# chalharu/rust-compression

Hardware: AMD Instinct MI355X
Metric: BZip2 level-9 encode MB/s (input bytes, HBM-resident in and out: the kernels' rate; value_end_to_end is host buffer to host buffer at the C ABI) (higher is better)
Workload: dtype u8/u32

## Files before the change

rust-compression_amd/csrc/bzgpu.h:

```cpp
#pragma once
#include <hip/hip_runtime.h>
#include <stdint.h>
#include <stddef.h>

namespace bzgpu {

typedef uint8_t u8;
typedef uint16_t u16;
typedef uint32_t u32;
typedef uint64_t u64;
typedef int64_t i64;

constexpr u32 kWave = 64;
constexpr u32 kMaxBlockLen = 900000;
constexpr u32 kSortTile = 8192;
constexpr u32 kSortThreads = 512;
constexpr u32 kTilesPerBlock = 110;
constexpr u32 kSlot = kTilesPerBlock * kSortTile;
constexpr u32 kPtSlot = kSlot / 8u * 10u;
constexpr u32 kPairWords = 65536u / 32u;
constexpr u32 kMaxBins = 2048;
constexpr u32 kPerK = 8;
constexpr u32 kGSize = 50;
constexpr u32 kMaxSelectors = 18002;
// ... 427 lines not shown
constexpr u32 kDecEntrySkip = 0xFFFFFFFFu;
struct DecEntry {
    u64 off, len;
    u32 first_cand, ncand;
};
enum : u32 { kChainOk = 0, kChainData = 1, kChainMagicFirst = 2, kChainMagic = 3 };
struct DecChainEntry {
    u32 verdict;
    u32 streams;
    u32 irregular;
    u32 ntrue;
};
struct DecChainCand {
    u32 is_true, max_len;
    u32 stored_crc, nsym;
};
void launch_dec_scan_batch(hipStream_t st, const u8 *in, u64 span0, u64 span_end, const DecEntry *ents, u32 nent,
                           DecCand *cands, u32 cap, u32 *count);
void launch_dec_blocks_batch(hipStream_t st, const u8 *in, const DecEntry *ents, const DecCand *cands, u32 ncand,
                             DecBlockInfo *info, u16 *sym, u8 *sel_scratch);
void launch_dec_chain_batch(hipStream_t st, const u8 *in, const DecEntry *ents, u32 e0, u32 ne, const DecCand *cands,
                            u32 cand0, const DecBlockInfo *info, DecChainEntry *out_ent, DecChainCand *out_cand);
void launch_dec_mtf(hipStream_t st, const DecArgs &a, KernelProf *prof, int *rec);
void launch_dec_gather_windows(hipStream_t st, const u8 *in, u64 nbytes, const u64 *bases, u32 nw, u8 *out);
void launch_dec_walks(hipStream_t st, const DecArgs &a, u32 walk_wgs, hipStream_t st2, hipEvent_t ev_a, hipEvent_t ev_b,
                      KernelProf *prof, int rec[4]);
void launch_dec_expand(hipStream_t st, const DecArgs &a, const u64 *out_base, u8 *out);
void launch_dec_crc(hipStream_t st, const DecArgs &a, const u64 *out_base, const u8 *out, u32 max_out_len,
                    const u32 *crc_tab, const u32 *xp2, const u32 *xp16);

enum KernelId {
    KID_RADIX_HIST = 0,
    KID_RADIX_SCAN,
    KID_RADIX_SCATTER,
    KID_GROUP_FLAGS,
    KID_GROUP_APPLY,
    KID_LAST_COLUMN,
    KID_RADIX_SCATTER_LB,
    KID_GHIST_TEXT,
    KID_GHIST_SCAN,
    KID_RANK_PLACE,
    KID_PHASE_B_LOCAL,
    KID_GROUP_REFINE,
    KID_DEC_BLOCK,
    KID_DEC_MTF,
    KID_DEC_TSORT,
    KID_DEC_WALK,
    KID_DEC_PLACE,
    KID_DEC_RLE,
    KID_DEC_CRC,
    KID_RLE_ONEPASS,
    KID_RLE_SCATTER,
    KID_MTF_HEADS,
    KID_COUNT
};
struct KernelProf {
    bool on = false;
    struct Rec {
        int id;
        u64 bytes;
        hipEvent_t a, b;
    };
    Rec *recs = nullptr;
    u32 nrecs = 0, cap = 0;
    u64 launches[KID_COUNT] = {};
    u64 bytes[KID_COUNT] = {};
    double seconds[KID_COUNT] = {};
    int begin(hipStream_t st, int id, u64 nbytes);
    void end(hipStream_t st, int idx);
    void set_bytes(int idx, u64 nbytes) { if (idx >= 0) recs[idx].bytes = nbytes; }
    void collect();
    void reset();
};

void launch_slab_last(hipStream_t st, const RleBuffers &rb, u64 t0, u64 t1, i64 *d_out);
void launch_rle_scan(hipStream_t st, const u8 *d_in, u64 n, u64 t0, u64 t1, u64 in_begin, const u32 *crc_tab,
                     const u32 *xp16, const RleBuffers &rb);
void launch_rle_count(hipStream_t st, const u8 *d_in, u64 n, u64 t0, u64 t1, u64 in_begin, i64 init_carry,
                      const RleBuffers &rb, i64 *d_out_last);
void launch_rle_prefix(hipStream_t st, u64 tb, u64 t1, const RleBuffers &rb, bool write_end = true);
void launch_rle_cuts(hipStream_t st, const u8 *d_in, u64 n, u64 tb, u64 t1, u64 in_begin, const RleBuffers &rb,
                     u32 block_max_len, int emit_tail, BlockDesc *d_blocks, u32 max_blocks);
void launch_rle_image(hipStream_t st, const u8 *d_in, u64 n, u64 tb, u64 t1, u64 in_begin, const RleBuffers &rb, u8 *d_rle);
u64 rle_onepass_spans(u64 ntiles);
u32 rle_onepass_epochs();
void launch_rle_onepass(hipStream_t st, const u8 *d_in, u64 n, u64 ntiles, u32 epoch, const u32 *crc_tab, const u32 *xp16,
                        const RleBuffers &rb, u8 *d_rle, i64 *d_out_last);
u64 cut_table_entries(const CutPlan &pl);
void cut_groups(const CutPlan &pl, u64 *g_lo, u64 *g_hi, u64 *entries);
u32 cut_seg_cap();
void launch_cut_steps(hipStream_t st, const CutPlan &pl, const RleBuffers &rb, const CutBuffers &cb);
void launch_cut_tables(hipStream_t st, const CutPlan &pl, const u8 *d_in, u64 n_lim, const RleBuffers &rb, const CutBuffers &cb,
                       u64 work_total);
void launch_cut_select(hipStream_t st, const CutPlan &pl, u64 j0, u64 s0, u64 start_in, u64 n, long long rle_bias, int emit_tail,
                       const RleBuffers &rb, const CutBuffers &cb, BlockDesc *d_blocks, u32 max_blocks);
void launch_block_crc(hipStream_t st, const u8 *d_in, const BlockDesc *d_blocks, u32 nblocks,
                      const u32 *crc_tab, const u32 *xp2, const u32 *tile_crc, u32 *d_crc);
void launch_rle_batch(hipStream_t st, const u8 *d_in, const RleBatchItem *d_items, u32 count, const u32 *crc_tab,
                      const u32 *xp2, u8 *d_rle, BlockDesc *d_blocks, u32 *d_crc);
void launch_block_symbols(hipStream_t st, const BwtArgs &a, u32 *inuse_bits, u8 *sym_code, u8 *keyinfo);
int run_bwt(hipStream_t st, const BwtArgs &a, u32 max_n, u64 total_n, unsigned long long *h_active,
            u64 *sorted_elems, KernelProf *prof, u64 *round_active , bool wide_keys,
            u32 min_chars);
void launch_mtf(hipStream_t st, const MtfArgs &a, KernelProf *prof = nullptr, u64 total_n = 0);
inline bool env_verify() { return getenv("BZ_VERIFY") && atoi(getenv("BZ_VERIFY")) != 0; }
struct MailSeg {
// ... 19 lines not shown
```

rust-compression_amd/csrc/engine.hip:

```cpp
#include "engine_state.h"

#include <algorithm>
#include <chrono>
#include <cstdio>
#include <cstdlib>
#include <cstring>
#include <vector>

#define MAILCHK(st, ...)                                                             \
    do {                                                                             \
        const MailSeg mail_segs_[] = {__VA_ARGS__};                                  \
        if (mail_fetch((st), mail_segs_, (int)(sizeof(mail_segs_) / sizeof(mail_segs_[0]))) != 0) return BZ_E_UNEXPECTED; \
    } while (0)

static int span_begin(bz_gpu_engine *g, int stage, hipStream_t st = nullptr)
{
    bz_gpu_engine::Span s;
    s.stage = stage;
    s.st = st ? st : g->st;
    if (hipEventCreate(&s.a) != hipSuccess || hipEventCreate(&s.b) != hipSuccess) return -1;
    (void)hipEventRecord(s.a, s.st);
    g->spans.push_back(s);
    return (int)g->spans.size() - 1;
}
// ... 1781 lines not shown
        if (bad) {
            fprintf(stderr, "bz2_mi355x: the one-launch ZLE stage misbehaved (tile tickets / look-back); stage redone with three kernels\n");
            g->zle_fused_broken = true;
            ma.fused_zle = 0;
            launch_mtf(g->st, ma, nullptr, total_n);
        }
    }
    std::vector<BlockOut> outs(nb);
    HIPCHK(hipMemcpyAsync(outs.data(), g->bout.p, nb * sizeof(BlockOut), hipMemcpyDeviceToHost, g->st));
    HIPCHK(hipMemcpyAsync(h_freq, g->mtf_freq.p, nb * kMaxAlpha * 4, hipMemcpyDeviceToHost, g->st));
    HIPCHK(hipStreamSynchronize(g->st));
    for (size_t i = 0; i < nb; ++i) {
        if (outs[i].mtf_count == 0 || outs[i].mtf_count > h_len[i] + 1u) return BZ_E_UNEXPECTED;
        h_mtf_count[i] = outs[i].mtf_count;
        h_in_use[i] = outs[i].in_use_count;
        HIPCHK(hipMemcpyAsync(h_sym + i * sym_stride, g->mtf.as<u16>() + i * kMtfStride, (size_t)outs[i].mtf_count * 2,
                              hipMemcpyDeviceToHost, g->st));
    }
    HIPCHK(hipStreamSynchronize(g->st));
    HIPCHK(hipGetLastError());
    return BZ_OK;
}

extern "C" int bz_gpu_debug_code_lengths(bz_gpu_engine *g, const uint32_t *h_freq, size_t alpha, uint8_t *h_len,
                                         int *took_length_limited_path)
{
    if (!g || alpha == 0 || alpha > kMaxAlpha) return BZ_E_PARAM;
    {
        uint64_t total = 0;
        for (size_t i = 0; i < alpha; ++i) total += h_freq[i] ? h_freq[i] : 1u;
        if (total >= (1u << 20)) return BZ_E_PARAM;
    }
    HIPCHK(hipSetDevice(g->device));
    DevBuf f, o, s, fl;
    int rc;
    if ((rc = f.ensure(alpha * 4)) || (rc = o.ensure(alpha + 8)) || (rc = s.ensure((size_t)kLmWords * 4)) ||
        (rc = fl.ensure(4)))
        return rc;
    HIPCHK(hipMemcpyAsync(f.p, h_freq, alpha * 4, hipMemcpyHostToDevice, g->st));
    launch_probe_code_lengths(g->st, f.as<u32>(), (u32)alpha, o.as<u8>(), s.as<u32>(), fl.as<int>());
    int flag = 0;
    HIPCHK(hipMemcpyAsync(h_len, o.p, alpha, hipMemcpyDeviceToHost, g->st));
    HIPCHK(hipMemcpyAsync(&flag, fl.p, 4, hipMemcpyDeviceToHost, g->st));
    HIPCHK(hipStreamSynchronize(g->st));
    HIPCHK(hipGetLastError());
    if (took_length_limited_path) *took_length_limited_path = flag;
    return BZ_OK;
}

static const char *kKernelNames[KID_COUNT] = {"k_radix_hist", "k_radix_scan", "k_radix_scatter",
                                              "k_group_flags", "k_group_apply", "k_last_column",
                                              "k_radix_scatter_lb", "k_ghist_text", "k_ghist_scan", "k_rank_place", "k_phase_b_local", "k_group_refine",
                                              "k_dec_block", "k_dec_mtf", "k_dec_tsort", "k_dec_walk_lengths",
                                              "k_dec_place", "k_dec_rle", "k_dec_crc", "k_rle_onepass", "k_rle_scatter", "k_mtf_heads"};

extern "C" int bz_gpu_profile_enable(bz_gpu_engine *g, int on)
{
    if (!g) return BZ_E_PARAM;
    g->prof.reset();
    g->prof.on = (on & 1) != 0;
    g->debug_figures = (on & 2) != 0;
    return BZ_OK;
}

extern "C" int bz_gpu_profile_kernels(bz_gpu_engine *g)
{
    (void)g;
    return KID_COUNT;
}

extern "C" int bz_gpu_profile_get(bz_gpu_engine *g, int idx, const char **name, uint64_t *launches,
                                  double *seconds, uint64_t *algorithmic_bytes)
{
    if (!g || idx < 0 || idx >= KID_COUNT) return BZ_E_PARAM;
    if (name) *name = kKernelNames[idx];
    if (launches) *launches = g->prof.launches[idx];
    if (seconds) *seconds = g->prof.seconds[idx];
    if (algorithmic_bytes) *algorithmic_bytes = g->prof.bytes[idx];
    return BZ_OK;
}
```

rust-compression_amd/csrc/k_bwt.hip:

```cpp
#include "bzgpu.h"
#include <algorithm>
#include <atomic>
#include <cstdio>
#include <cstdlib>
#include <vector>

namespace bzgpu {
constexpr u32 kGhSpan = 8;
constexpr u32 kSymSpan = 8;

enum { SRC_TEXT = 0, SRC_PAIRS = 1, SRC_MM = 2, SRC_WALK = 3, SRC_SURV = 4, SRC_LISTG = 5,
       SRC_TEXTK = 6, SRC_WALKK = 7, SRC_MMK = 8,
       SRC_MMC = 9,
       SRC_PERJ = 10,
       SRC_PACKED = 11,
       SRC_PERJK = 12,
       SRC_WALKA = 13 };
template <int SRC> struct src_is_list {
    static constexpr bool value = (SRC == SRC_PAIRS || SRC == SRC_SURV || SRC == SRC_LISTG || SRC == SRC_PERJ || SRC == SRC_PERJK || SRC == SRC_PACKED);
};

struct KeyInfo {
    u8 bits;
    u8 chars;
// ... 972 lines not shown
}

__device__ __forceinline__ void loc_fill(u64 (&e)[16], const u64 *s_e, u32 pos0, u32 len, u32 l, u64 le_mask, u32 gshift,
                                         u32 &gcarry)
{
#pragma unroll
    for (u32 r = 0; r < 16; ++r) {
        const u32 i = pos0 + r * 64u + l;
        const u64 x = s_e[i < len ? i : len - 1u];
        const u64 m = __ballot(i < len && (x >> 63) != 0);
        const u32 gi = gcarry + (u32)__popcll(m & le_mask) - 1u;
        e[r] = (x & ~(1ull << 63)) | ((u64)gi << gshift);
        gcarry += (u32)__popcll(m);
    }
}
__device__ __forceinline__ void loc_rank(const u64 (&e)[16], u32 (&rnk)[16], u32 *cnt, u32 pos0, u32 len, u32 l, u32 shift)
{
#pragma unroll
    for (u32 q = 0; q < kLocBins / 2 / 64; ++q) cnt[q * 64u + l] = 0;
#pragma unroll
    for (u32 r = 0; r < 16; ++r) {
        const u32 i = pos0 + r * 64u + l;
        const u32 dg = (u32)(e[r] >> shift) & (kLocBins - 1u);
        const u32 sh = (dg & 1u) * 16u;
        u32 old = 0;
        if (i < len)
            old = __hip_atomic_fetch_add(cnt + (dg >> 1), 1u << sh, __ATOMIC_RELAXED, __HIP_MEMORY_SCOPE_WORKGROUP);
        rnk[r] = (old >> sh) & 0xFFFFu;
    }
}
__device__ __forceinline__ void loc_move(const u64 (&e)[16], const u32 (&rnk)[16], const u32 *cnt, const u16 *s_tpre,
                                         u64 *s_e, u32 pos0, u32 len, u32 l, u32 shift)
{
    const u16 *c16 = reinterpret_cast<const u16 *>(cnt);
#pragma unroll
    for (u32 r = 0; r < 16; ++r) {
        const u32 i = pos0 + r * 64u + l;
        const u32 dg = (u32)(e[r] >> shift) & (kLocBins - 1u);
        const u32 to = (u32)s_tpre[dg] + (u32)c16[dg] + rnk[r];
        if (i < len) s_e[to] = e[r];
    }
}
__device__ __forceinline__ void loc_reload(u64 (&e)[16], const u64 *s_e, u32 pos0, u32 len, u32 l)
{
#pragma unroll
    for (u32 r = 0; r < 16; ++r) {
        const u32 i = pos0 + r * 64u + l;
        e[r] = s_e[i < len ? i : len - 1u];
    }
}

#define LOC_T(k) do { } while (0)
constexpr u32 LOC_STAT_SURV_FAIL = 80;
__device__ __forceinline__ u32 first_group_start_list(const u32 *__restrict__ R, const u32 *__restrict__ Vb, u32 p0, u32 cnt, u32 limit)
{
    if (p0 == 0) return 0;
    if (p0 >= cnt) return cnt;
    const u32 l = threadIdx.x & 63u;
    for (u32 q0 = p0; q0 < p0 + limit; q0 += 64u) {
        if (q0 >= cnt) return cnt;
        const u32 q = q0 + l;
        bool b = false;
        if (q < cnt) b = (R[Vb[q] & 0xFFFFFu] & ~kFinalBit) != (R[Vb[q - 1] & 0xFFFFFu] & ~kFinalBit);
        const u64 m = __ballot(b);
        if (m) return q0 + (u32)__ffsll((long long)m) - 1u;
    }
    return 0xFFFFFFFFu;
}
__global__ __launch_bounds__(kLocThreads) void k_surv_local(BwtArgs a, u32 step, const u32 *__restrict__ V, u32 *__restrict__ Kout,
                                                             u32 *__restrict__ Vout)
{
    __shared__ u64 s_e[kLocCap];
    __shared__ u32 s_cnt[kLocSets][kLocBins / 2];
    __shared__ u16 s_tpre[kLocBins];
    __shared__ u32 s_wsum[kLocSets];
    __shared__ u32 s_seg[2];
    __shared__ u32 s_bad;
    u32 tile, lb;
    xcd_remap(gridDim.x, a.nb, tile, lb);
    if (lb == 0xFFFFFFFFu) return;
    const u32 n = a.blocks[lb].n;
    const u32 cnt = a.count[lb];
    const u32 start = tile * kSortTile;
    if (start >= cnt) return;
    const KeyInfo ki = reinterpret_cast<const KeyInfo *>(a.keyinfo)[lb];
    const u32 hm = (((u32)ki.chars * 2u) << step) % n;
    const size_t base = (size_t)lb * kSlot;
    const u32 *Rb = a.R + base, *Vl = V + base;
    const u32 w = threadIdx.x >> 6, l = threadIdx.x & 63u;
    if (w == 0) {
        const u32 s = first_group_start_list(Rb, Vl, start, cnt, kLocCap + 64u);
        if (l == 0) s_seg[0] = s;
    } else if (w == 1) {
        const u32 s = first_group_start_list(Rb, Vl, start + kSortTile, cnt, kLocCap + 64u);
        if (l == 0) s_seg[1] = s;
    }
    if (threadIdx.x == 0) s_bad = 0;
    __syncthreads();
    const u32 s0 = (u32)__builtin_amdgcn_readfirstlane((int)s_seg[0]), s1 = (u32)__builtin_amdgcn_readfirstlane((int)s_seg[1]);
    if (s0 == 0xFFFFFFFFu || s1 == 0xFFFFFFFFu || (s1 > s0 && s1 - s0 > kLocCap)) {
        if (threadIdx.x == 0) atomicAdd(&a.loc_stats[LOC_STAT_SURV_FAIL], 1u);
        return;
    }
    if (s1 <= s0) return;
    const u32 len = s1 - s0;
    const u32 *Vb = Vl + s0;
    const u32 wu = (u32)__builtin_amdgcn_readfirstlane((int)w);
    const u32 posA = wu * 1024u, posB = kSortTile + wu * 1024u;
    u32 gcount[2] = {0, 0};
#pragma unroll 1
    for (u32 half = 0; half < 2; ++half) {
        const u32 pos0 = half ? posB : posA;
        if (pos0 >= len) break;
        u32 prev_last = 0;
        if (l == 0 && pos0 > 0) prev_last = Rb[Vb[pos0 - 1u] & 0xFFFFFu] & ~kFinalBit;
        const u32 rows = (len - pos0 + 63u) / 64u < 16u ? (len - pos0 + 63u) / 64u : 16u;
        u32 tot = 0;
#pragma unroll 4
        for (u32 r = 0; r < rows; ++r) {
            const u32 i = pos0 + r * 64u + l;
            const u32 c = i < len ? i : len - 1u;
            const u32 v = ld_stream(Vb + c) & 0xFFFFFu;
// ... 23 lines not shown
        groups += c;
    }
    const u64 le_mask = (l == 63) ? ~0ull : ((2ull << l) - 1ull);
    constexpr u32 kbits = 20u;
    const u32 gshift = 20u + kbits;
    const bool haveB = posB < len;
    u64 eA[16], eB[16];
    loc_fill(eA, s_e, posA, len, l, le_mask, gshift, gcarryA);
    if (haveB) loc_fill(eB, s_e, posB, len, l, le_mask, gshift, gcarryB);
    const u32 gbits = groups > 1u ? 32u - (u32)__builtin_clz(groups - 1u) : 0u;
    const u32 npass = (kbits + gbits + kLocBits - 1u) / kLocBits;
    u32 *cntA = s_cnt[w], *cntB = s_cnt[kLocWaves + w];
    u16 *cnt16 = reinterpret_cast<u16 *>(&s_cnt[0][0]);
#pragma unroll 1
    for (u32 p = 0; p < npass; ++p) {
        const u32 shift = 20u + p * kLocBits;
        u32 rnkA[16], rnkB[16];
        loc_rank(eA, rnkA, cntA, posA, len, l, shift);
        if (haveB) loc_rank(eB, rnkB, cntB, posB, len, l, shift);
        else {
#pragma unroll
            for (u32 q = 0; q < kLocBins / 2 / 64; ++q) cntB[q * 64u + l] = 0;
        }
        __syncthreads();
        u32 tot;
        {
            const u32 dg = threadIdx.x;
            u32 run = 0;
#pragma unroll
            for (u32 k = 0; k < kLocSets; ++k) {
                const u32 c = cnt16[k * kLocBins + dg];
                cnt16[k * kLocBins + dg] = (u16)run;
                run += c;
            }
            tot = run;
        }
        const u32 inc = wave_incl_sum(tot);
        if (l == 63) s_wsum[w] = inc;
        __syncthreads();
        {
            u32 carry = 0;
            for (u32 k = 0; k < w; ++k) carry += s_wsum[k];
            s_tpre[threadIdx.x] = (u16)(carry + inc - tot);
        }
        __syncthreads();
        loc_move(eA, rnkA, cntA, s_tpre, s_e, posA, len, l, shift);
        if (haveB) loc_move(eB, rnkB, cntB, s_tpre, s_e, posB, len, l, shift);
        __syncthreads();
        if (p + 1 < npass) {
            loc_reload(eA, s_e, posA, len, l);
            if (haveB) loc_reload(eB, s_e, posB, len, l);
        }
    }
    {
        bool bad = false;
        for (u32 i = threadIdx.x; i < len; i += kLocThreads) {
            const u64 x = s_e[i];
            if (i && (s_e[i - 1] >> 20) > (x >> 20)) bad = true;
            const u32 v = (u32)x & 0xFFFFFu;
            Vout[base + s0 + i] = v;
            Kout[base + s0 + i] = Rb[v] & ~kFinalBit;
        }
        if (__ballot(bad) && l == 0) s_bad = 1u;
    }
    __syncthreads();
    if (threadIdx.x == 0 && s_bad) atomicAdd(&a.loc_stats[LOC_STAT_SURV_FAIL], 1u);
}

template <bool INIT>
__global__ __launch_bounds__(kSortThreads) void k_group_flags(BwtArgs a, u32 step, const u32 *__restrict__ K,
                                                               const u32 *__restrict__ V,
                                                               const u8 *__restrict__ impure = nullptr)
{
    __shared__ int s_old, s_new;
    u32 tile, lb;
    xcd_remap(gridDim.x, a.nb, tile, lb);
    if (lb == 0xFFFFFFFFu) return;
    const BlockDesc d = a.blocks[lb];
    const u32 n = d.n;
    const u32 cnt = a.count[lb];
    const u32 start = tile * kSortTile;
    if (start >= cnt) return;
    const KeyInfo ki = reinterpret_cast<const KeyInfo *>(a.keyinfo)[lb];
    const u32 hm = INIT ? (u32)ki.chars % n : (((u32)ki.chars * 2u) << step) % n;
    const u8 *text = a.rle + d.rle_off;
    const u8 *pt = a.ptext + (size_t)lb * kPtSlot;
    const size_t base = (size_t)lb * kSlot;
    if (INIT && a.pb_gate[lb] == 0u) K = a.KA;
    if (threadIdx.x == 0) {
        s_old = -1;
        s_new = -1;
    }
    __syncthreads();
    const u32 w = threadIdx.x >> 6, l = threadIdx.x & 63u;
    int last_old = -1, last_new = -1;
    const u32 first = start + w * 1024u + l;
    u32 g[16], s1[16], s2[16];
    u32 pg0 = 0, ps10 = 0, ps20 = 0;
    {
        u32 jj[16];
#pragma unroll
        for (u32 r = 0; r < 16; ++r) {
            const u32 idx = first + r * 64u;
            const u32 c = idx < cnt ? idx : cnt - 1u;
            const u32 kk = ld_stream(K + base + c);
            const u32 t = ld_stream(V + base + c) + hm;
// ... 28 lines not shown
            if (need_prev) {
                const u32 jr = pj >= hm ? pj - hm : pj + n - hm;
                const u32 im = impure[base + pg0];
                u32 ek;
                ps10 = (im == 2u || (per && im == 0u)) ? jr + 1u : ((per && a.per_wide && per_ekey(a, lb, text, n, depth, jr, ek)) ? ek + 1u : 0u);
            }
        } else {
#pragma unroll
            for (u32 r = 0; r < 16; ++r) s1[r] = a.R[base + jj[r]];
            if (need_prev) ps10 = a.R[base + pj];
        }
    }
#pragma unroll
    for (u32 r = 0; r < 16; ++r) {
        const u32 idx = first + r * 64u;
        const bool ok = idx < cnt;
        u32 pg = wave_shr1(g[r]), p1 = wave_shr1(s1[r]), p2 = wave_shr1(s2[r]);
        const u32 qg = (r == 0) ? pg0 : wave_lane(g[(r + 15) & 15], 63);
        const u32 q1 = (r == 0) ? ps10 : wave_lane(s1[(r + 15) & 15], 63);
        const u32 q2 = (r == 0) ? ps20 : wave_lane(s2[(r + 15) & 15], 63);
        if (l == 0) {
            pg = qg;
            p1 = q1;
            p2 = q2;
        }
        bool ns = false;
        if (ok) {
            const bool os = (idx == 0) || (g[r] != pg);
            ns = os || (s1[r] != p1) || (s2[r] != p2);
            a.flags[base + idx] = (u8)((os ? 1u : 0u) | (ns ? 2u : 0u));
            if (os) last_old = (int)idx;
            if (ns) last_new = (int)idx;
        }
        const u64 mrow = __ballot(ns);
        if (l == 0 && idx < cnt) a.newbits[(base + idx) >> 6] = mrow;
    }
#pragma unroll
    for (u32 dd = 32; dd >= 1; dd >>= 1) {
        const int o1 = __shfl_xor(last_old, dd, 64), o2 = __shfl_xor(last_new, dd, 64);
        last_old = o1 > last_old ? o1 : last_old;
        last_new = o2 > last_new ? o2 : last_new;
    }
    if (l == 0) {
        if (last_old >= 0) atomicMax(&s_old, last_old);
        if (last_new >= 0) atomicMax(&s_new, last_new);
    }
    __syncthreads();
    if (threadIdx.x == 0) {
        a.tile_last_old[lb * kTilesPerBlock + tile] = s_old;
        a.tile_last_new[lb * kTilesPerBlock + tile] = s_new;
    }
}

constexpr u32 kRankBinShift = 10, kRankBins = kSlot >> kRankBinShift;
constexpr u32 kRankBinSize = 1u << kRankBinShift, kRankBinMask = kRankBinSize - 1u;
static_assert(kRankBinShift + 20u + 1u <= 32u, "j inside the bin, a 20-bit head and the final bit share a word");
static_assert(kRankBins <= 1024 && (kRankBins << kRankBinShift) == kSlot, "bins tile the slot");

template <bool INIT>
__global__ __launch_bounds__(kSortThreads) void k_group_apply(BwtArgs a, u32 next_step, u32 round,
                                                               const u32 *__restrict__ K,
                                                               const u32 *__restrict__ V,
                                                               u32 *__restrict__ W)
{
    constexpr u32 NW = kSortThreads / 64;
    __shared__ int s_carry_old, s_carry_new;
    __shared__ int s_wold[NW], s_wnew[NW];
    __shared__ u32 s_nonfinal;
    __shared__ u32 s_gh[2][1024];
    __shared__ u32 s_stage[kSortTile];
    __shared__ u16 s_binof[kSortTile];
    __shared__ u32 s_bcnt[1024];
    __shared__ u16 s_bpre[1024];
    __shared__ u32 s_wsum[NW];
    u32 tile, lb;
    xcd_remap(gridDim.x, a.nb, tile, lb);
    if (lb == 0xFFFFFFFFu) return;
    const BlockDesc d = a.blocks[lb];
    const u32 n = d.n;
    const u8 *__restrict__ text = a.rle + d.rle_off;
    const u32 cnt = a.count[lb];
    const u32 start = tile * kSortTile;
    if (start >= cnt) return;
    const size_t base = (size_t)lb * kSlot;
    if (a.fused)
        for (u32 i = threadIdx.x; i < 2048u; i += kSortThreads) (&s_gh[0][0])[i] = 0;
    for (u32 i = threadIdx.x; i < 1024u; i += kSortThreads) s_bcnt[i] = 0;

    if (threadIdx.x == 0) {
        int co = -1, cn = -1;
        for (int t = (int)tile - 1; t >= 0 && co < 0; --t) co = a.tile_last_old[lb * kTilesPerBlock + t];
        for (int t = (int)tile - 1; t >= 0 && cn < 0; --t) cn = a.tile_last_new[lb * kTilesPerBlock + t];
        s_carry_old = co;
        s_carry_new = cn;
        s_nonfinal = 0;
    }
    const u32 w = threadIdx.x >> 6, l = threadIdx.x & 63u;
    const u32 wbase = start + w * 1024u;
    u32 gk[16], jv[16];
#pragma unroll
    for (u32 r = 0; r < 16; ++r) {
        const u32 idx = wbase + r * 64u + l;
        const u32 c = idx < cnt ? idx : cnt - 1u;
        gk[r] = INIT ? 0u : ld_stream(K + base + c);
        jv[r] = ld_stream(V + base + c);
    }
    u64 mo[16], mn[16];
    int wl_old = -1, wl_new = -1;
#pragma unroll
    for (u32 r = 0; r < 16; ++r) {
// ... 1746 lines not shown
    const bool refine = fused && want_refine;
    int p;
    (void)hipMemsetAsync(a.bin_cursor, 0, (size_t)a.nb * 1024 * sizeof(u32), st);
    if (refine) {
        const u32 e = next_epoch(st, a);
        p = prof ? prof->begin(st, KID_GROUP_REFINE, abits ? total_n * 10 + total_n / 8 : total_n * 14) : -1;
        if (abits) hipLaunchKernelGGL((k_group_refine<true, true>), grid, dim3(kSortThreads), 0, st, a, 0u, 0u, 0u, (const u32 *)nullptr, a.SA, a.KA, e);
        else hipLaunchKernelGGL((k_group_refine<true>), grid, dim3(kSortThreads), 0, st, a, 0u, 0u, 0u, a.KB, a.SA, a.KA, e);
        if (prof) prof->end(st, p);
    } else {
        p = prof ? prof->begin(st, KID_GROUP_FLAGS, total_n * 9) : -1;
        hipLaunchKernelGGL((k_group_flags<true>), grid, dim3(kSortThreads), 0, st, a, 0u, a.KB, a.SA);
        if (prof) prof->end(st, p);
        p = prof ? prof->begin(st, KID_GROUP_APPLY, total_n * 13) : -1;
        hipLaunchKernelGGL((k_group_apply<true>), grid, dim3(kSortThreads), 0, st, a, 0u, 0u, a.KB, a.SA, a.KA);
        if (prof) prof->end(st, p);
    }
    p = prof ? prof->begin(st, KID_RANK_PLACE, total_n * 8) : -1;
    hipLaunchKernelGGL(k_rank_place, grid, dim3(kSortThreads), 0, st, a, a.KA);
    if (prof) prof->end(st, p);

    u32 *cK = a.KB, *cV = a.VB;
    u32 *fK = a.KA, *fV = a.VA;
    const u32 *lastV = a.SA;
    u32 step = 0;
    int rounds = 0;
    u32 slot = 0;
    bool period_done = false;
    bool last_doubled = false, links_pay = true;
    u64 link_m = 0;
    if (!(a.gh_tiles && a.per_aux)) a.per_links = 0;
    const u32 links_on = a.per_links;
    bool surv_local_ok = true;
    u32 list_tiles = a.tiles;
    while (true) {
        {
            const MailSeg sg[2] = {{h_active, a.active + slot, sizeof(unsigned long long)}, {h_active + 1, a.maxnf + slot, sizeof(u32)}};
            if (mail_fetch(st, sg, 2) != 0) return -1;
        }
        const u64 m = *h_active;
        const u32 list_tiles_prev = list_tiles;
        const u32 mx = *reinterpret_cast<const u32 *>(h_active + 1);
        {
            list_tiles = (mx + kSortTile - 1) / kSortTile + 1u;
            if (list_tiles > kTilesPerBlock) list_tiles = kTilesPerBlock;
        }
        const dim3 grid_list(list_tiles, xcd_grid_y(a.nb)), grid_prev(list_tiles_prev, xcd_grid_y(a.nb));
        if (sorted_elems) *sorted_elems += m;
        if (round_active && slot < 64) round_active[slot] += m;
        if (m == 0 || step > 24 || ((u64)(2u * min_chars) << step) >= max_n) break;
        ++slot;
        ++rounds;
        bool carried = false;
        u32 trace_worst = 0;
        static const bool bwt_trace = getenv("BZ_BWT_TRACE") != nullptr;
        if (bwt_trace) {
            std::vector<u32> nf(a.nb);
            (void)hipMemcpyAsync(nf.data(), a.nonfinal, a.nb * 4, hipMemcpyDeviceToHost, st);
            (void)hipStreamSynchronize(st);
            trace_worst = (u32)(std::max_element(nf.begin(), nf.end()) - nf.begin());
        }
        (void)hipMemsetAsync(a.nonfinal, 0, a.nb * sizeof(u32), st);
        static const int want_period = [] {
            const char *e = getenv("BZ_PERIOD_ROUND");
            return !e ? 1 : (e[0] == 'b' ? 2 : (atoi(e) != 0 ? 1 : 0));
        }();
        const bool deep = want_period == 2 ? (rounds >= 3 && m * 4 >= total_n * 3)
                                           : ((rounds >= 2 && ((u64)mx * 4 >= (u64)max_n * 3 || m * 4 >= total_n * 3)) ||
                                              (rounds == 1 && m * 64 >= total_n * 63));
        const bool per_round = want_period != 0 && !period_done && deep;
        if (link_m) {
            if ((link_m - m) * 4 < link_m) links_pay = false;
            link_m = 0;
        }
        const bool link_round = !per_round && links_on && period_done && last_doubled && links_pay && m * 256 >= total_n;
        constexpr u64 surv_num = 1, surv_den = 4;
        if (bwt_trace)
            fprintf(stderr, "bz2_mi355x: sort round %d (h = %llu): %llu of %llu rotations unordered, at most %u in one block (block %u; of %u)%s\n",
                    rounds, (unsigned long long)(2u * min_chars) << step, (unsigned long long)m, (unsigned long long)total_n, mx,
                    trace_worst, max_n, per_round ? ": period round" : (link_round ? ": link round" : (m * surv_den < total_n * surv_num ? ": survivor form" : ": walk form")));
        u8 *impure = a.ptext;
        last_doubled = !(per_round || link_round);
        if (per_round || link_round) {
            if (per_round) period_done = true;
            else link_m = m;
            (void)hipMemsetAsync(impure, 0, (size_t)a.nb * kSlot, st);
            const bool links = links_on != 0 && !(per_round && rounds == 1);
            a.per_links = links ? 1u : 0u;
            u32 *midx = cK;
            if (links) (void)hipMemsetAsync(midx, 0, (size_t)a.nb * kSlot * sizeof(u32), st);
            hipLaunchKernelGGL(k_survivor_compact, grid_prev, dim3(kSortThreads), 0, st, a, lastV, fV, links ? midx : nullptr, per_round ? 1u : 0u);
            hipLaunchKernelGGL(k_copy_counts, dim3((a.nb + 255) / 256), dim3(256), 0, st, a.count, a.count2, a.nb);
            if (links) hipLaunchKernelGGL(k_link_scan, grid, dim3(kSortThreads), 0, st, a, step, fV, midx, impure, fK);
            if (links) hipLaunchKernelGGL(k_link_finalize, grid_list, dim3(kSortThreads), 0, st, a, fV, impure, fK);
            if (link_round) {
                (void)hipMemsetAsync(a.lin_p, 0, (size_t)a.nb * kPerK * 4, st);
                hipLaunchKernelGGL(k_link_compact, grid_list, dim3(kSortThreads), 0, st, a, fV, cK, cV);
            } else {
            hipLaunchKernelGGL(k_period_find, dim3(a.nb), dim3(kSortThreads), 0, st, a, 3u);
            hipLaunchKernelGGL(k_period_bits, grid, dim3(kSortThreads), 0, st, a);
            hipLaunchKernelGGL(k_period_next, dim3(a.nb, per_kmax(a)), dim3(kSortThreads), 0, st, a);
            bool one_pass = false, wide = false;
            {
                std::vector<u32> lp((size_t)a.nb * kPerK), ls((size_t)a.nb * kPerK);
                {
                    const MailSeg sg[2] = {{lp.data(), a.lin_p, lp.size() * 4}, {ls.data(), a.lin_sig, ls.size() * 4}};
                    if (mail_fetch(st, sg, 2) != 0) return -1;
                }
                one_pass = true;
                u32 small = 0, smallest = 0xFFFFFFFFu;
                const u64 depth_max = 16ull << step;
                for (size_t i = 0; i < lp.size(); ++i) {
                    if (lp[i] != 0u && lp[i] < 1024u && ls[i] >= 200u) {
                        one_pass = false;
                        small += 1;
                        smallest = lp[i] < smallest ? lp[i] : smallest;
                    }
                    if (lp[i] != 0u && lp[i] <= depth_max) wide = true;
                }
                if (wide) one_pass = false;
                if (bwt_trace) fprintf(stderr, "  period round: %s (%u distances below 1024 that a fifth of their block agrees at, the smallest %u)\n", wide ? "three passes over thirty-bit keys" : (one_pass ? "one pass over the keys" : "two passes over the keys"), small, small ? smallest : 0u);
            }
            a.per_keyshift = one_pass ? 10u : 0u;
            a.per_wide = wide ? 1u : 0u;
            if (one_pass) {
                radix_pass<SRC_PERJ, 10>(st, a, 0, step, nullptr, fV, cK, cV, m, prof, fK, list_tiles);
                radix_pass<SRC_LISTG, 10>(st, a, 0, step, nullptr, cV, fK, cK, m, prof, fV, list_tiles);
                radix_pass<SRC_PAIRS, 10>(st, a, 10, step, fK, cK, cV, fV, m, prof, nullptr, list_tiles);
                u32 *rk = cV, *rv = fV, *ok = fK, *ov = cK;
                cK = rk; cV = rv; fK = ok; fV = ov;
            } else if (wide) {
                radix_pass<SRC_PERJ, 10>(st, a, 0, step, nullptr, fV, cK, cV, m, prof, fK, list_tiles);
                radix_pass<SRC_PAIRS, 10>(st, a, 10, step, cK, cV, fK, fV, m, prof, nullptr, list_tiles);
                radix_pass<SRC_PAIRS, 10>(st, a, 20, step, fK, fV, cK, cV, m, prof, nullptr, list_tiles);
                radix_pass<SRC_LISTG, 10>(st, a, 0, step, nullptr, cV, fK, fV, m, prof, cK, list_tiles);
                radix_pass<SRC_PAIRS, 10>(st, a, 10, step, fK, fV, cK, cV, m, prof, nullptr, list_tiles);
            } else {
                radix_pass<SRC_PERJ, 10>(st, a, 0, step, nullptr, fV, cK, cV, m, prof, fK, list_tiles);
                radix_pass<SRC_PAIRS, 10>(st, a, 10, step, cK, cV, fK, fV, m, prof, nullptr, list_tiles);
                radix_pass<SRC_LISTG, 10>(st, a, 0, step, nullptr, fV, cK, cV, m, prof, fK, list_tiles);
                radix_pass<SRC_PAIRS, 10>(st, a, 10, step, cK, cV, fK, fV, m, prof, nullptr, list_tiles);
                u32 *t = cK; cK = fK; fK = t;
                t = cV; cV = fV; fV = t;
            }
            a.per_keyshift = 0;
            hipLaunchKernelGGL(k_period_mark, grid_list, dim3(kSortThreads), 0, st, a, step, cK, cV, impure);
            }
        } else if (m * surv_den < total_n * surv_num) {
            hipLaunchKernelGGL(k_survivor_compact, grid_prev, dim3(kSortThreads), 0, st, a, lastV, fV);
            hipLaunchKernelGGL(k_copy_counts, dim3((a.nb + 255) / 256), dim3(256), 0, st, a.count, a.count2, a.nb);
            bool local_done = false;
            if (surv_local_ok && m * 8 < total_n) {
                u32 fails = 0;
                (void)hipMemsetAsync(a.loc_stats + LOC_STAT_SURV_FAIL, 0, 4, st);
                hipLaunchKernelGGL(k_surv_local, grid_list, dim3(kLocThreads), 0, st, a, step, fV, cK, cV);
                {
                    const MailSeg sg = {&fails, a.loc_stats + LOC_STAT_SURV_FAIL, 4};
                    if (mail_fetch(st, &sg, 1) != 0) return -1;
                }
                local_done = fails == 0;
                if (!local_done) surv_local_ok = false;
                if (bwt_trace) fprintf(stderr, "  survivor round inside LDS: %s\n", local_done ? "done" : "a segment did not fit or failed its check: the global passes");
            }
            if (!local_done) {
            radix_pass<SRC_SURV, 10>(st, a, 0, step, nullptr, fV, cK, cV, m, prof, fK, list_tiles);
            radix_pass<SRC_PAIRS, 10>(st, a, 10, step, cK, cV, fK, fV, m, prof, nullptr, list_tiles);
            radix_pass<SRC_LISTG, 10>(st, a, 0, step, nullptr, fV, cK, cV, m, prof, fK, list_tiles);
            radix_pass<SRC_PAIRS, 10>(st, a, 10, step, cK, cV, fK, fV, m, prof, nullptr, list_tiles);
            u32 *t = cK; cK = fK; fK = t;
            t = cV; cV = fV; fV = t;
            }
        } else {
            if (fused) {
                hipLaunchKernelGGL(k_ghist_scan, dim3(a.nb), dim3(kSortThreads), 0, st, a, 2u, 1024u, 1024u, 0u, 1u);
                carried = refine && rounds == 1;
                if (carried) fused_pass<SRC_MMC, 10>(st, a, 0, step, nullptr, nullptr, fK, fV, 0, total_n, prof, m);
                else fused_pass<SRC_MM, 10>(st, a, 0, step, nullptr, nullptr, fK, fV, 0, total_n, prof, m);
                fused_pass<SRC_PAIRS, 10>(st, a, 10, step, fK, fV, cK, cV, 1, m, prof);
            } else {
                radix_pass<SRC_MM, 10>(st, a, 0, step, nullptr, nullptr, fK, fV, total_n, prof, cK);
                radix_pass<SRC_PAIRS, 10>(st, a, 10, step, fK, fV, cK, cV, m, prof);
            }
        }
        (void)hipMemsetAsync(a.bin_cursor, 0, (size_t)a.nb * 1024 * sizeof(u32), st);
        if (per_round || link_round) {
            p = prof ? prof->begin(st, KID_GROUP_FLAGS, m * 13) : -1;
            hipLaunchKernelGGL((k_group_flags<false>), grid_list, dim3(kSortThreads), 0, st, a, step, cK, cV, impure);
            a.per_wide = 0;
            a.per_links = links_on;
            if (prof) prof->end(st, p);
            p = prof ? prof->begin(st, KID_GROUP_APPLY, m * 17) : -1;
            hipLaunchKernelGGL((k_group_apply<false>), grid_list, dim3(kSortThreads), 0, st, a, step, slot, cK, cV, fK);
            if (prof) prof->end(st, p);
        } else if (carried) {
            const u32 e = next_epoch(st, a);
            p = prof ? prof->begin(st, KID_GROUP_REFINE, m * 18) : -1;
            hipLaunchKernelGGL((k_group_refine<false>), grid, dim3(kSortThreads), 0, st, a, step, step + 1, slot, cK, cV, fK, e);
            if (prof) prof->end(st, p);
        } else {
            p = prof ? prof->begin(st, KID_GROUP_FLAGS, m * 13) : -1;
            hipLaunchKernelGGL((k_group_flags<false>), grid_list, dim3(kSortThreads), 0, st, a, step, cK, cV);
            if (prof) prof->end(st, p);
            p = prof ? prof->begin(st, KID_GROUP_APPLY, m * 17) : -1;
            hipLaunchKernelGGL((k_group_apply<false>), grid_list, dim3(kSortThreads), 0, st, a, step + 1, slot, cK, cV, fK);
            if (prof) prof->end(st, p);
        }
        p = prof ? prof->begin(st, KID_RANK_PLACE, m * 8) : -1;
        hipLaunchKernelGGL(k_rank_place, grid, dim3(kSortThreads), 0, st, a, fK);
        if (prof) prof->end(st, p);
        if (per_round && bwt_trace) {
            std::vector<u32> lp((size_t)a.nb * kPerK), ls((size_t)a.nb * kPerK), nf(a.nb), cn(a.nb);
            (void)hipMemcpyAsync(lp.data(), a.lin_p, (size_t)a.nb * kPerK * 4, hipMemcpyDeviceToHost, st);
            (void)hipMemcpyAsync(ls.data(), a.lin_sig, (size_t)a.nb * kPerK * 4, hipMemcpyDeviceToHost, st);
            (void)hipMemcpyAsync(nf.data(), a.nonfinal, a.nb * 4, hipMemcpyDeviceToHost, st);
            (void)hipMemcpyAsync(cn.data(), a.count, a.nb * 4, hipMemcpyDeviceToHost, st);
            (void)hipStreamSynchronize(st);
            for (u32 b = 0; b < a.nb; ++b)
                if (lp[(size_t)b * kPerK] || nf[b] * 2u > max_n) {
                    fprintf(stderr, "  block %u: distances (agreement in permille of the block)", b);
                    for (u32 i = 0; i < kPerK && lp[(size_t)b * kPerK + i]; ++i) fprintf(stderr, " %u (%u)", lp[(size_t)b * kPerK + i], ls[(size_t)b * kPerK + i]);
                    fprintf(stderr, "; list %u, %u rotations left unordered\n", cn[b], nf[b]);
                }
        }
        lastV = cV;
        if (!per_round && !link_round) ++step;
    }
    if (fused) {
        u32 gave_up = 0;
        std::vector<u32> tk;
        const u32 epoch_last = *a.epoch;
        if (epoch_last >= epoch_first)
            tk.resize((size_t)(epoch_last - epoch_first + 1u) * 8u);
        {
            const MailSeg sg[2] = {{&gave_up, a.sort_err, 4}, {tk.data(), a.tickets + (size_t)epoch_first * 8u, tk.size() * 4}};
            if (mail_fetch(st, sg, tk.empty() ? 1 : 2) != 0) return -1;
        }
        static const bool late_fail_test = getenv("BZ_ONESWEEP_LATEFAILTEST") != nullptr;
        bool bad = gave_up != 0 || late_fail_test;
// ... 68 lines not shown
```

Baseline: 15080.

## Fuse group flag and apply work into the LDS survivor-sort kernel

```diff
diff --git a/rust-compression_amd/csrc/bzgpu.h b/rust-compression_amd/csrc/bzgpu.h
--- a/rust-compression_amd/csrc/bzgpu.h
+++ b/rust-compression_amd/csrc/bzgpu.h
@@ -503,6 +503,7 @@
     KID_RLE_ONEPASS,
     KID_RLE_SCATTER,
     KID_MTF_HEADS,
+    KID_SURV_LOCAL,
     KID_COUNT
 };
 struct KernelProf {
diff --git a/rust-compression_amd/csrc/engine.hip b/rust-compression_amd/csrc/engine.hip
--- a/rust-compression_amd/csrc/engine.hip
+++ b/rust-compression_amd/csrc/engine.hip
@@ -1857,7 +1857,7 @@
                                               "k_group_flags", "k_group_apply", "k_last_column",
                                               "k_radix_scatter_lb", "k_ghist_text", "k_ghist_scan", "k_rank_place", "k_phase_b_local", "k_group_refine",
                                               "k_dec_block", "k_dec_mtf", "k_dec_tsort", "k_dec_walk_lengths",
-                                              "k_dec_place", "k_dec_rle", "k_dec_crc", "k_rle_onepass", "k_rle_scatter", "k_mtf_heads"};
+                                              "k_dec_place", "k_dec_rle", "k_dec_crc", "k_rle_onepass", "k_rle_scatter", "k_mtf_heads", "k_surv_local"};
 
 extern "C" int bz_gpu_profile_enable(bz_gpu_engine *g, int on)
 {
diff --git a/rust-compression_amd/csrc/k_bwt.hip b/rust-compression_amd/csrc/k_bwt.hip
--- a/rust-compression_amd/csrc/k_bwt.hip
+++ b/rust-compression_amd/csrc/k_bwt.hip
@@ -1048,6 +1048,10 @@
 
 #define LOC_T(k) do { } while (0)
 constexpr u32 LOC_STAT_SURV_FAIL = 80;
+constexpr u32 kRankBinShift = 10, kRankBins = kSlot >> kRankBinShift;
+constexpr u32 kRankBinSize = 1u << kRankBinShift, kRankBinMask = kRankBinSize - 1u;
+static_assert(kRankBinShift + 20u + 1u <= 32u, "j inside the bin, a 20-bit head and the final bit share a word");
+static_assert(kRankBins <= 1024 && (kRankBins << kRankBinShift) == kSlot, "bins tile the slot");
 __device__ __forceinline__ u32 first_group_start_list(const u32 *__restrict__ R, const u32 *__restrict__ Vb, u32 p0, u32 cnt, u32 limit)
 {
     if (p0 == 0) return 0;
@@ -1063,7 +1067,102 @@
     }
     return 0xFFFFFFFFu;
 }
-__global__ __launch_bounds__(kLocThreads) void k_surv_local(BwtArgs a, u32 step, const u32 *__restrict__ V, u32 *__restrict__ Kout,
+__device__ __forceinline__ void surv_scan(const u64 *s_e, u64 *s_bits, u32 pos0, u32 len, u32 l, u64 le_mask, u32 (&vj)[16],
+                                          u32 (&meta)[16], int &last_old, int &last_new)
+{
+    int co = -1, cn = -1;
+    u64 edge = pos0 ? s_e[pos0 - 1u] : 0ull;
+#pragma unroll
+    for (u32 r = 0; r < 16; ++r) {
+        const u32 rowbase = pos0 + r * 64u, i = rowbase + l;
+        const bool ok = i < len;
+        const u64 x = s_e[ok ? i : len - 1u];
+        const u64 nx = s_e[i + 1u < len ? i + 1u : len - 1u];
+        u64 px = ((u64)wave_shr1((u32)(x >> 32)) << 32) | wave_shr1((u32)x);
+        if (l == 0) px = edge;
+        edge = wave_lane64(x, 63);
+        const bool os = ok && (i == 0 || (x >> 40) != (px >> 40));
+        const bool ns = ok && (i == 0 || (x >> 20) != (px >> 20));
+        const bool fin = ns && (i + 1u >= len || (nx >> 20) != (x >> 20));
+        const u64 mo = __ballot(os), mn = __ballot(ns);
+        if (l == 0 && rowbase < len) s_bits[rowbase >> 6] = mn;
+        const u64 o = mo & le_mask, q = mn & le_mask;
+        const int rs = o ? (int)(rowbase + 63u - __clzll(o)) : co;
+        const int ss = q ? (int)(rowbase + 63u - __clzll(q)) : cn;
+        vj[r] = (u32)x & 0xFFFFFu;
+        meta[r] = ((u32)rs & 0x3FFFu) | (((u32)ss & 0x3FFFu) << 14) | (fin ? 1u << 28 : 0u) | (ok ? 1u << 29 : 0u) |
+                  (rs < 0 ? 1u << 30 : 0u) | (ss < 0 ? 1u << 31 : 0u);
+        if (mo) co = (int)(rowbase + 63u - __clzll(mo));
+        if (mn) cn = (int)(rowbase + 63u - __clzll(mn));
+    }
+    last_old = co;
+    last_new = cn;
+}
+__device__ __forceinline__ void surv_heads(u64 *s_e, const u32 *__restrict__ Rb, const u8 *__restrict__ text, u32 n, u32 pos0, u32 l,
+                                           const u32 (&vj)[16], const u32 (&meta)[16], u32 (&lc)[4])
+{
+#pragma unroll
+    for (u32 r = 0; r < 16; ++r) {
+        const u32 m = meta[r], j = vj[r];
+        u32 c = 0;
+        if ((m & (3u << 28)) == (3u << 28)) c = text[j ? j - 1u : n - 1u];
+        lc[r >> 2] |= c << ((r & 3u) * 8u);
+    }
+#pragma unroll
+    for (u32 r = 0; r < 16; ++r) {
+        const u32 i = pos0 + r * 64u + l, m = meta[r];
+        if ((m & (3u << 29)) == (1u << 29) && (m & 0x3FFFu) == i) s_e[i] = (u64)vj[r] | ((u64)(Rb[vj[r]] & ~kFinalBit) << 20);
+    }
+}
+__device__ __forceinline__ void surv_apply(const BwtArgs &a, u32 lb, size_t base, const u64 *s_e, u32 *s_bcnt, u32 *__restrict__ Vout,
+                                           u32 pos0, u32 l, u32 s0, int co, int cn, u32 (&vj)[16], u32 (&meta)[16],
+                                           const u32 (&lc)[4], u32 (&nf)[3])
+{
+    const u32 t0 = s0 / kSortTile;
+#pragma unroll
+    for (u32 r = 0; r < 16; ++r) {
+        const u32 i = pos0 + r * 64u + l, m = meta[r], j = vj[r];
+        u32 word = 0, pk = 0xFFFFFFFFu;
+        if (m & (1u << 29)) {
+            const u32 rs = (m & (1u << 30)) ? (u32)co : (m & 0x3FFFu);
+            const u32 ss = (m & (1u << 31)) ? (u32)cn : ((m >> 14) & 0x3FFFu);
+            const bool fin = (m & (1u << 28)) != 0;
+            const u32 g = (u32)(s_e[rs] >> 20) & 0xFFFFFu;
+            const u32 p = g + (i - rs);
+            const u32 head = g + (ss - rs);
+            st_stream(a.SA + base + p, j);
+            Vout[base + s0 + i] = j;
+            if (fin) {
+                a.L[base + p] = (u8)(lc[r >> 2] >> ((r & 3u) * 8u));
+                if (j == 0) a.orig_ptr[lb] = p;
+            }
+            word = (j & kRankBinMask) | (head << kRankBinShift) | (fin ? kFinalBit : 0u);
+            pk = (j >> kRankBinShift) | (atomicAdd(&s_bcnt[j >> kRankBinShift], 1u) << 10);
+            if (!fin) {
+                const u32 t = (s0 + i) / kSortTile - t0;
+                nf[0] += t == 0u ? 1u : 0u;
+                nf[1] += t == 1u ? 1u : 0u;
+                nf[2] += t == 2u ? 1u : 0u;
+            }
+        }
+        meta[r] = word;
+        vj[r] = pk;
+    }
+}
+__device__ __forceinline__ void surv_stage(u32 *s_stage, u16 *s_binof, const u16 *s_bpre, const u32 (&vj)[16], const u32 (&meta)[16])
+{
+#pragma unroll
+    for (u32 r = 0; r < 16; ++r) {
+        if (vj[r] != 0xFFFFFFFFu) {
+            const u32 bin = vj[r] & 1023u;
+            const u32 pos = (u32)s_bpre[bin] + (vj[r] >> 10);
+            s_stage[pos] = meta[r];
+            s_binof[pos] = (u16)bin;
+        }
+    }
+}
+template <bool FUSED>
+__global__ __launch_bounds__(kLocThreads) void k_surv_local(BwtArgs a, u32 step, u32 round, const u32 *__restrict__ V, u32 *__restrict__ Kout,
                                                              u32 *__restrict__ Vout)
 {
     __shared__ u64 s_e[kLocCap];
@@ -1193,6 +1292,128 @@
             if (haveB) loc_reload(eB, s_e, posB, len, l);
         }
     }
+    if (FUSED) {
+        {
+            bool bad = false;
+            for (u32 i = threadIdx.x; i < len; i += kLocThreads)
+                if (i && (s_e[i - 1] >> 20) > (s_e[i] >> 20)) bad = true;
+            if (__ballot(bad) && l == 0) s_bad = 1u;
+        }
+        u32 *sc = &s_cnt[0][0];
+        u32 *s_bcnt = sc;
+        u16 *s_bpre = reinterpret_cast<u16 *>(sc + 1024);
+        u64 *s_bits = reinterpret_cast<u64 *>(sc + 2048);
+        int *s_wold = reinterpret_cast<int *>(sc + 3072), *s_wnew = s_wold + kLocSets;
+        u32 *s_tnf = sc + 3072 + 2 * kLocSets;
+        static_assert(kLocSets * kLocBins / 2 >= 3072 + 2 * kLocSets + 4 && kLocCap / 64 * 2 <= 1024, "the scratch of the fused form fits the counters");
+        for (u32 i = threadIdx.x; i < 1024u; i += kLocThreads) s_bcnt[i] = 0;
+        if (threadIdx.x < 4u) s_tnf[threadIdx.x] = 0;
+        __syncthreads();
+        if (s_bad) {
+            if (threadIdx.x == 0) atomicAdd(&a.loc_stats[LOC_STAT_SURV_FAIL], 1u);
+            return;
+        }
+        const BlockDesc d = a.blocks[lb];
+        const u8 *__restrict__ text = a.rle + d.rle_off;
+        u32 vA[16], mA[16], vB[16], mB[16];
+        int loA = -1, lnA = -1, loB = -1, lnB = -1;
+        surv_scan(s_e, s_bits, posA, len, l, le_mask, vA, mA, loA, lnA);
+        if (haveB) surv_scan(s_e, s_bits, posB, len, l, le_mask, vB, mB, loB, lnB);
+        else {
+#pragma unroll
+            for (u32 r = 0; r < 16; ++r) {
+                vB[r] = 0;
+                mB[r] = 0;
+            }
+        }
+        if (l == 0) {
+            s_wold[w] = loA;
+            s_wnew[w] = lnA;
+            s_wold[kLocWaves + w] = loB;
+            s_wnew[kLocWaves + w] = lnB;
+        }
+        __syncthreads();
+        u32 lcA[4] = {0, 0, 0, 0}, lcB[4] = {0, 0, 0, 0};
+        surv_heads(s_e, Rb, text, n, posA, l, vA, mA, lcA);
+        if (haveB) surv_heads(s_e, Rb, text, n, posB, l, vB, mB, lcB);
+        int coA = -1, cnA = -1, coB = -1, cnB = -1;
+        for (u32 k = 0; k < kLocSets; ++k) {
+            const int o = s_wold[k], q = s_wnew[k];
+            if (k < w) {
+                coA = o > coA ? o : coA;
+                cnA = q > cnA ? q : cnA;
+            }
+            if (k < kLocWaves + w) {
+                coB = o > coB ? o : coB;
+                cnB = q > cnB ? q : cnB;
+            }
+        }
+        __syncthreads();
+        u32 nf[3] = {0, 0, 0};
+        surv_apply(a, lb, base, s_e, s_bcnt, Vout, posA, l, s0, coA, cnA, vA, mA, lcA, nf);
+        if (haveB) surv_apply(a, lb, base, s_e, s_bcnt, Vout, posB, l, s0, coB, cnB, vB, mB, lcB, nf);
+#pragma unroll
+        for (u32 k = 0; k < 3; ++k) {
+            const u32 c = wave_sum(nf[k]);
+            if (l == 0 && c) atomicAdd(&s_tnf[k], c);
+        }
+        __syncthreads();
+        if (threadIdx.x < 3u && s_tnf[threadIdx.x]) atomicAdd(&a.tile_nf[lb * kTilesPerBlock + s0 / kSortTile + threadIdx.x], s_tnf[threadIdx.x]);
+        if (threadIdx.x == 0) {
+            const u32 tot = s_tnf[0] + s_tnf[1] + s_tnf[2];
+            if (tot) {
+                atomicMax(&a.maxnf[round], atomicAdd(&a.nonfinal[lb], tot) + tot);
+                const u32 h_next = ((u32)ki.chars * 2u) << (step + 1u);
+                if (h_next < n) atomicAdd(&a.active[round], (unsigned long long)tot);
+            }
+        }
+        {
+            const u32 q0 = s0 >> 6, sh = s0 & 63u, nwords = ((s1 - 1u) >> 6) - q0 + 1u, nrel = (len + 63u) >> 6;
+            for (u32 t = threadIdx.x; t < nwords; t += kLocThreads) {
+                const u64 cur = t < nrel ? s_bits[t] : 0ull, prv = t ? s_bits[t - 1u] : 0ull;
+                const u64 val = sh ? ((cur << sh) | (prv >> (64u - sh))) : cur;
+                const u32 lo = t ? 0u : sh;
+                const u32 hi = (t + 1u == nwords && s1 != cnt) ? ((s1 - 1u) & 63u) + 1u : 64u;
+                const u64 mask = (~0ull << lo) & (hi == 64u ? ~0ull : ~(~0ull << hi));
+                unsigned long long *dst = reinterpret_cast<unsigned long long *>(a.newbits + (base >> 6) + q0 + t);
+                if (mask == ~0ull) *dst = val;
+                else {
+                    atomicAnd(dst, (unsigned long long)~mask);
+                    atomicOr(dst, (unsigned long long)(val & mask));
+                }
+            }
+        }
+        {
+            const u32 b0 = threadIdx.x * 2u;
+            const u32 c0 = s_bcnt[b0], c1 = s_bcnt[b0 + 1];
+            const u32 mine = c0 + c1;
+            const u32 inc = wave_incl_sum(mine);
+            if (l == 63) s_wsum[w] = inc;
+            u32 g0 = 0, g1 = 0;
+            u32 *cur = a.bin_cursor + (size_t)lb * 1024u;
+            if (c0) g0 = atomicAdd(&cur[b0], c0);
+            if (c1) g1 = atomicAdd(&cur[b0 + 1], c1);
+            __syncthreads();
+            u32 carry = 0;
+            for (u32 k = 0; k < w; ++k) carry += s_wsum[k];
+            const u32 ex = carry + inc - mine;
+            s_bpre[b0] = (u16)ex;
+            s_bpre[b0 + 1] = (u16)(ex + c0);
+            s_bcnt[b0] = (b0 << kRankBinShift) + g0;
+            s_bcnt[b0 + 1] = ((b0 + 1u) << kRankBinShift) + g1;
+        }
+        __syncthreads();
+        u32 *s_stage = reinterpret_cast<u32 *>(s_e);
+        u16 *s_binof = reinterpret_cast<u16 *>(s_stage + kLocCap);
+        surv_stage(s_stage, s_binof, s_bpre, vA, mA);
+        if (haveB) surv_stage(s_stage, s_binof, s_bpre, vB, mB);
+        __syncthreads();
+        for (u32 i = threadIdx.x; i < len; i += kLocThreads) {
+            const u32 bin = s_binof[i];
+            Kout[base + s_bcnt[bin] + (i - (u32)s_bpre[bin])] = s_stage[i];
+        }
+        return;
+    }
     {
         bool bad = false;
         for (u32 i = threadIdx.x; i < len; i += kLocThreads) {
@@ -1327,10 +1548,6 @@
     }
 }
 
-constexpr u32 kRankBinShift = 10, kRankBins = kSlot >> kRankBinShift;
-constexpr u32 kRankBinSize = 1u << kRankBinShift, kRankBinMask = kRankBinSize - 1u;
-static_assert(kRankBinShift + 20u + 1u <= 32u, "j inside the bin, a 20-bit head and the final bit share a word");
-static_assert(kRankBins <= 1024 && (kRankBins << kRankBinShift) == kSlot, "bins tile the slot");
 
 template <bool INIT>
 __global__ __launch_bounds__(kSortThreads) void k_group_apply(BwtArgs a, u32 next_step, u32 round,
@@ -3183,6 +3400,7 @@
         ++slot;
         ++rounds;
         bool carried = false;
+        bool refined = false;
         u32 trace_worst = 0;
         static const bool bwt_trace = getenv("BZ_BWT_TRACE") != nullptr;
         if (bwt_trace) {
@@ -3281,16 +3499,31 @@
             hipLaunchKernelGGL(k_survivor_compact, grid_prev, dim3(kSortThreads), 0, st, a, lastV, fV);
             hipLaunchKernelGGL(k_copy_counts, dim3((a.nb + 255) / 256), dim3(256), 0, st, a.count, a.count2, a.nb);
             bool local_done = false;
+            static const bool want_surv_fused = !(getenv("BZ_SURV_FUSED") && atoi(getenv("BZ_SURV_FUSED")) == 0);
             if (surv_local_ok && m * 8 < total_n) {
                 u32 fails = 0;
                 (void)hipMemsetAsync(a.loc_stats + LOC_STAT_SURV_FAIL, 0, 4, st);
-                hipLaunchKernelGGL(k_surv_local, grid_list, dim3(kLocThreads), 0, st, a, step, fV, cK, cV);
+                p = prof ? prof->begin(st, KID_SURV_LOCAL, m * (want_surv_fused ? 25 : 20)) : -1;
+                if (want_surv_fused) {
+                    (void)hipMemsetAsync(a.bin_cursor, 0, (size_t)a.nb * 1024 * sizeof(u32), st);
+                    (void)hipMemsetAsync(a.tile_nf, 0, (size_t)a.nb * kTilesPerBlock * sizeof(u32), st);
+                    hipLaunchKernelGGL((k_surv_local<true>), grid_list, dim3(kLocThreads), 0, st, a, step, slot, fV, fK, cV);
+                } else {
+                    hipLaunchKernelGGL((k_surv_local<false>), grid_list, dim3(kLocThreads), 0, st, a, step, slot, fV, cK, cV);
+                }
+                if (prof) prof->end(st, p);
                 {
                     const MailSeg sg = {&fails, a.loc_stats + LOC_STAT_SURV_FAIL, 4};
                     if (mail_fetch(st, &sg, 1) != 0) return -1;
                 }
                 local_done = fails == 0;
                 if (!local_done) surv_local_ok = false;
+                refined = local_done && want_surv_fused;
+                if (!local_done && want_surv_fused) {
+                    (void)hipMemsetAsync(a.nonfinal, 0, a.nb * sizeof(u32), st);
+                    (void)hipMemsetAsync(a.active + slot, 0, sizeof(unsigned long long), st);
+                    (void)hipMemsetAsync(a.maxnf + slot, 0, sizeof(u32), st);
+                }
                 if (bwt_trace) fprintf(stderr, "  survivor round inside LDS: %s\n", local_done ? "done" : "a segment did not fit or failed its check: the global passes");
             }
             if (!local_done) {
@@ -3313,8 +3546,9 @@
                 radix_pass<SRC_PAIRS, 10>(st, a, 10, step, fK, fV, cK, cV, m, prof);
             }
         }
-        (void)hipMemsetAsync(a.bin_cursor, 0, (size_t)a.nb * 1024 * sizeof(u32), st);
-        if (per_round || link_round) {
+        if (!refined) (void)hipMemsetAsync(a.bin_cursor, 0, (size_t)a.nb * 1024 * sizeof(u32), st);
+        if (refined) {
+        } else if (per_round || link_round) {
             p = prof ? prof->begin(st, KID_GROUP_FLAGS, m * 13) : -1;
             hipLaunchKernelGGL((k_group_flags<false>), grid_list, dim3(kSortThreads), 0, st, a, step, cK, cV, impure);
             a.per_wide = 0;
```

Result: no change. 15150 (median of 6 runs) (+0.5%).
